# r3fang/alignTools.C

Measured on AMD Instinct MI355X. Metric: GCUPS (DP cell updates/s), SW affine-gap 150bp pairs, higher is better.
Workload: dtype int16; 1 GPU; C2: local affine-gap, 100000 x (150x150 bp) pairs per GPU, uniform ACGT, m=2 u=-2 o=-5 e=-2, scores+tracebacks+rendered strings; pairs_per_gpu=100000, l1=150, l2=150, bits_per_base=2, streams=3, parallelism=pairs sharded over 1 GPU(s), one process per GPU

## Files before the change

### aligntools/c_amd/csrc/at_hip.hip

```cpp
#include "at_launch.h"
#include "at_classes.h"
#include "at_ragplan.h"
#include "at_pack.hip.h"
#include "at_render.hip.h"
#include "at_myers.hip.h"
#include "at_search.hip.h"
#include "at_revcomp.hip.h"
#include "at_cigar.hip.h"
#include "at_edit_tb.hip.h"
#include "../../../include/aligntools_hip.h"

#include <algorithm>
#include <chrono>
#include <condition_variable>
#include <mutex>
#include <cstdarg>
#include <cstdio>
#include <cstdlib>
#include <cstring>
#include <functional>
#include <string>
#include <thread>
#include <vector>

// ... 475 lines not shown
		L.g = 16;
		L.k = at::class_rows(at::kClass16, l1);
	} else if ((force_g == 16 || (!force_g && g_forced != 64 && g_forced != 32)) && ts == 4 && l1 > 208 && l1 <= at::class_top(at::kClass16)) {
		L.g = 16;
		L.k = at::class_rows(at::kClass16, l1);
	} else if (g_forced != 64 && ts == 4 && l1 > 208 &&
	           l1 <= (force_g || g_forced == 32 ? at::kTopFit : kmode == at::K_LOCAL ? at::kTopLocal : kmode == at::K_GLOBAL ? at::kTopGlobal : at::kTopFit)) {
		L.g = 32;
		L.k = at::class_rows(at::kClass32, l1, 0, g_forced == 32 ? at::kClass32SkipUnderGroup32 : 0);
	}
	const int ng = 64 / L.g;
	const int blk = L.g <= 16 ? 4 : 8;
	const int tbk = (l2 + L.g - 1 + blk - 1) / blk;
	L.ptr_lanes = L.g == 64 ? std::max(1, std::min(64, (l1 + L.k - 1) / L.k)) : 64;
	L.ptr_lanes = (L.ptr_lanes + 3) & ~3;
	const long long nstrips = (l1 + L.g * L.k - 1) / (L.g * L.k);
	long long nref = (at::kPad + (long long)tbk * blk) / 4 + 4;
	nref = (nref + 1) & ~1LL;
	const long long walk_words = ((L.k + 3) / 4 + (hasj ? ((L.k + 3) / 4 + 3) / 4 : 0)) * (long long)at::ck_steps(L.g);
	const long long nbound = std::max<long long>(2LL * (l2 + 2), two_pass == 1 ? std::max<long long>(at::ck_stage_words(at::ck_steps(L.g)), 2 * ng * walk_words * (L.g == 64 ? 4 : 1)) : 0);
	const int spw = overlap ? 16 / AT_OVL_BITS : (hasj && !(ts == 4 && AT_JPLANE)) ? 2 : 4;
	const long long njpl = tb && hasj && ts == 4 && AT_JPLANE ? nstrips * tbk * (blk / 4) * ((L.k + 3) / 4) * L.ptr_lanes : 0;
	const long long nptr = tb ? nstrips * tbk * (blk / spw) * L.k * L.ptr_lanes + njpl + 64 : 0;
	const long long nsm = hasj ? (((long long)l2 + 64 + 64 + 128 + 31) / 32 + 2 + 1) & ~1LL : 0;
	L.off_refb = (int)nref;
	L.off_bound = (int)(2 * nref * ng);
	L.off_sm = (int)(2 * nref * ng + nbound);
	L.nsm = (int)nsm;
	L.off_ptr = (int)((2 * nref * ng + nbound + nsm + 3) & ~3LL);
	L.words = L.off_ptr + nptr;
	return L;
}

static bool packed_ok(const at_handle *h, int mode, int bits, int l1, int l2, int ts, int *thresh16)
{
	const long long scale = 1LL << ts;
	if (getenv("AT_NO_PACKED") && atoi(getenv("AT_NO_PACKED"))) return false;
	if ((bits != 2 && bits != 8) || l1 < 1 || l2 < 1) return false;
	if (mode == AT_MODE_OVERLAP) {
		if (ts != 2 || h->m < 0 || h->u > 0 || h->o > 0) return false;
		const long long lo = std::llabs((long long)h->o) * std::max(l1, l2) + std::llabs((long long)h->u) + 16;
		const long long hi = (long long)h->m * std::min(l1, l2), slack = std::llabs((long long)h->o) + std::llabs((long long)h->u) + 3;
		if (scale * (lo + hi + slack) >= 32768) return false;
		*thresh16 = (int)(-32768 + scale * (hi + slack));
		return true;
	}
	if (!(mode == AT_MODE_GLOBAL || mode == AT_MODE_LOCAL || mode == AT_MODE_FIT)) return false;
	if (h->m < 0 || h->u > 0 || h->o > 0 || h->e > 0) return false;
	const bool hasj = mode == AT_MODE_FIT && h->use_jump;
	if (hasj && (h->j > 0 || std::llabs((long long)h->j - h->o) * scale > 32000)) return false;
	const long long A = std::max<long long>(std::max(std::llabs((long long)h->e), std::llabs((long long)h->u)), h->m);
	(void)A;
	long long lo = 3 * std::llabs((long long)h->o) + (hasj ? std::llabs((long long)h->j) : 0) +
	               std::llabs((long long)h->u) * std::min(l1, l2) + std::llabs((long long)h->e) * std::max(l1, l2) + 16;
	if (mode == AT_MODE_LOCAL) lo = std::llabs((long long)h->o) + std::llabs((long long)h->u) + std::llabs((long long)h->e) + 16;
	const long long hi = (long long)h->m * std::min(l1, l2);
	const long long slack = std::llabs((long long)h->o) + std::llabs((long long)h->e) + 3;
	if (scale * (lo + hi + slack) >= 32768) return false;
	*thresh16 = (int)(-32768 + scale * (hi + slack));
	return true;
}

struct TpLayout {
	int off_brow, off_rck, off_cck, off_rptr, off_rjpl;
	long long words;
	long long brow_words;
};
static TpLayout tp_layout(const Layout16 &L, int kmode, int l2, bool split = false)
{
	const int blk = L.g <= 16 ? 4 : 8, cb = at::ck_steps(L.g);
	const long long T = (long long)((l2 + L.g - 1 + blk - 1) / blk) * blk;
	const int es = 2, nq = ((kmode == at::K_FITJ ? 3 : 2) * L.k + 3) / 4, kg = (L.k + 3) / 4;
	auto up4 = [](long long v) { return (v + 3) & ~3LL; };
	TpLayout t;
	long long w = 0;
	t.brow_words = (T + cb + 2) * es;
	t.off_brow = (int)w; if (!split) w = up4(w + (T + cb + 2) * es);
	t.off_rck = (int)w; w = up4(w + 64 * es + (T / cb + 3) * 64 * cb * es);
	t.off_cck = (int)w; w = up4(w + (T / cb + 3) * ((nq + AT_CK_COL_QUAD - 1) / AT_CK_COL_QUAD * AT_CK_COL_QUAD) * 256);
	t.off_rptr = (int)w; if (!split) w = up4(w + (cb / 4) * ((L.k + 3) / 4) * 256);
	t.off_rjpl = (int)w; if (!split) w = up4(w + (cb / 4) * ((kg + 3) / 4) * 256);
	t.words = split ? (w + 63) & ~63LL : w;
	return t;
}

static int choose_store(long long words_fixed, long long words_ptr, bool prefer_hbm_pointers);
static bool packed16_kernel_exists(int kmode, const Layout16 &P, bool tb, int ts, int bits, int rag, const Layout16 *PT = nullptr)
{
	const long long fixed = PT ? std::max(P.off_ptr, PT->off_ptr) : P.off_ptr;
	const long long ptrw = PT ? std::max(P.words - P.off_ptr, PT->words - PT->off_ptr) : P.words - P.off_ptr;
	const int st = choose_store(fixed, ptrw, P.g < 64 || rag);
// ... 298 lines not shown
	drop_stale_error();

	long long maxabs = 0;
	for (int v : {h->m, h->u, h->o, h->e, h->j}) maxabs = std::max<long long>(maxabs, std::llabs((long long)v));
	maxabs = std::max<long long>(maxabs, 1);
	if (maxabs * ((long long)max_len1 + max_len2 + 2) >= (1LL << 24))
		return fail(h, AT_ERR_RANGE, "scores may exceed the exact range: max|param|=%lld, l1+l2=%lld", maxabs,
		            (long long)max_len1 + max_len2);

	h->last_span = max_len1 + max_len2;
	const int kmode = mode == AT_MODE_GLOBAL ? at::K_GLOBAL : mode == AT_MODE_LOCAL ? at::K_LOCAL
	                : mode == AT_MODE_FIT ? (h->use_jump ? at::K_FITJ : at::K_FIT)
	                : mode == AT_MODE_OVERLAP ? at::K_OVERLAP : at::K_EDIT;

	int thresh16 = 0, ts = 0;
	if (!uniform_shape && !rag && !only_if && ap_n == 0 && npairs >= 4096 && !d_order && kmode <= at::K_FITJ &&
	    env_ll("AT_AUTO_UNIFORM", 1) && (bits == 8 || scores_fit_byte(h, mode)) &&
	    packed_ok(h, mode, bits, max_len1, max_len2, 4, &thresh16)) {
		int *flag = h->d_rflag + 8;
		HIP_TRY(h, hipMemsetAsync(flag, 0xff, 4, stream));
		const unsigned cg = (unsigned)std::min<int64_t>((npairs + 255) / 256, 4LL * h->ncu);
		hipLaunchKernelGGL(at::at_check_uniform, dim3(cg), dim3(256), 0, stream, d_len1, d_len2, (long long)npairs, max_len1, max_len2, flag);
		int rc = align_device(h, mode, npairs, d_seq, bits, d_woff1, d_len1, d_woff2, d_len2, max_len1, max_len2, 1, want_traceback,
		                      d_score, d_end_i, d_end_j, d_state, d_ops, d_ops_off, d_nops, stream_, 0, 0, nullptr, 0, flag, -1);
		if (rc) return rc;
		std::string packed_cfg = h->cfg;
		rc = align_device(h, mode, npairs, d_seq, bits, d_woff1, d_len1, d_woff2, d_len2, max_len1, max_len2, 0, want_traceback,
		                  d_score, d_end_i, d_end_j, d_state, d_ops, d_ops_off, d_nops, stream_, 0, 0, nullptr, 0, flag, 0);
		if (rc) return rc;
		snprintf(h->cfg, sizeof h->cfg, "auto: [%.140s] if every pair is %dx%d, else [%.120s]", packed_cfg.c_str(), max_len1, max_len2,
		         std::string(h->cfg).c_str());
		return AT_OK;
	}
	if ((uniform_shape || rag) && ap_n == 0) {
		if (packed_ok(h, mode, bits, max_len1, max_len2, 4, &thresh16)) ts = 4;
		else if ((!rag || kmode == at::K_OVERLAP) && packed_ok(h, mode, bits, max_len1, max_len2, 2, &thresh16)) ts = 2;
		if (kmode == at::K_OVERLAP && (!tb || getenv("AT_NO_PACKED_OVERLAP"))) ts = 0;
	}
	if (rag && (!ts || (kmode > at::K_FITJ && !(kmode == at::K_OVERLAP && rag == 64)) || max_len1 > at::rag_group_top(rag) || !d_order))
		return fail(h, AT_ERR_ARG, "ragged packed launch outside its domain");
	Layout16 P;
	if (ts) {
		P = layout16_for(tb, kmode == at::K_FITJ, max_len1, max_len2, ts, rag, kmode == at::K_OVERLAP, kmode,
		                 rag && kmode == at::K_OVERLAP ? at::class_rows(at::kClassOvl, max_len1) : 0);
		const double min_rounds = getenv("AT_PACKED_MIN_ROUNDS") ? atof(getenv("AT_PACKED_MIN_ROUNDS")) : 1.0;
		if (!rag && P.g == 64 && (double)((npairs + 1) / 2) < min_rounds * 12.0 * h->ncu) ts = 0;
		if (P.words >= (1LL << 24)) { if (rag) return fail(h, AT_ERR_ARG, "ragged packed launch outside its domain (slot too large)"); ts = 0; }
		Layout16 PTq = P;
		const bool tailq = !rag && !only_if && P.g <= 16 && kmode != at::K_OVERLAP && env_ll("AT_TAIL_SPLIT", 1);
		if (tailq) PTq = layout16_for(tb, kmode == at::K_FITJ, max_len1, max_len2, ts, at::AT_TAIL_G, false, kmode, at::at_tail_k(P.g, P.k));
		if (ts && !packed16_kernel_exists(kmode, P, tb, ts, bits, rag, tailq ? &PTq : nullptr)) {
			if (rag) return fail(h, AT_ERR_ARG, "ragged packed launch outside its domain (frame too long for LDS)");
			ts = 0;
		}
	}
	bool two_pass = false;
	int tp_split = 0;
	const char *ck_note = "";
	const long long tp_mode = env_ll("AT_TWO_PASS", 1);
	if (ts && tb && !rag && kmode <= at::K_FITJ && tp_mode) {
		Layout16 P2 = layout16_for(false, kmode == at::K_FITJ, max_len1, max_len2, ts, 0, false, kmode, 0, 1);
		const bool narrow_default = P2.g == 8 && tp_split_narrow_default(kmode, max_len1, max_len2);
		const bool split_default = P2.g == 64 || narrow_default;
		const bool split_want = env_ll("AT_TP_SPLIT", split_default ? 1 : 0) && at_pick_walk16(kmode, P2.g, P2.k, ts, bits);
		const int split_req = split_want && !h->ck_alloc_failed && !h->ck_skip ? 1 : 0;
		if (split_want && !split_req) ck_note = h->ck_skip ? " [one work item's checkpoints exceed AT_CK_CAP_MB: no separate pass 2]"
		                                                   : " [checkpoint buffer unavailable on this handle: no separate pass 2]";
		if ((P2.g == 64 || tp_mode >= 2 || (split_req && narrow_default)) && (long long)P2.g * P2.k >= max_len1 && at_pick16_tp(kmode, P2.g, P2.k, ts, bits) &&
		    choose_store(P2.off_ptr, 1, true) == 1) {
			two_pass = true;
			tp_split = split_req;
			if (tp_split) P2 = layout16_for(false, kmode == at::K_FITJ, max_len1, max_len2, ts, 0, false, kmode, 0, 2);
			P = P2;
		}
	}
	if (ts) {
		const int per_wave = 2 * (64 / P.g);
		const bool tail_ok = !rag && !only_if && P.g <= 16 && kmode != at::K_OVERLAP && env_ll("AT_TAIL_SPLIT", 1) &&
		                     (!tp_split || P.g == 8);
		Layout16 PT = P;
		if (tail_ok) PT = layout16_for(tb && !two_pass, kmode == at::K_FITJ, max_len1, max_len2, ts, at::AT_TAIL_G, false, kmode, at::at_tail_k(P.g, P.k), two_pass ? (tp_split ? 2 : 1) : 0);
		TpLayout tpm{}, tpt{};
		if (two_pass) { tpm = tp_layout(P, kmode, max_len2, tp_split != 0); tpt = tp_layout(PT, kmode, max_len2, tp_split != 0); }
		int64_t piece = npairs;
		int64_t brow_words = 0;
		if (tp_split) {
			const long long cap = env_ll("AT_CK_CAP_MB", 8192) << 20;
			brow_words = (tpm.brow_words + 63) & ~63LL;
			const long long tail_reserve = tail_ok ? 16LL * h->ncu * tpt.words * 4 : 0;
			const long long items = (cap - tail_reserve - brow_words * 4) / (tpm.words * 4 + 16LL * per_wave);
			if (items < 1) {
				struct SkipForThisCall {
					at_handle *h;
					explicit SkipForThisCall(at_handle *hh) : h(hh) { h->ck_skip = true; }
					~SkipForThisCall() { h->ck_skip = false; }
				} skip(h);
				return align_device(h, mode, npairs, d_seq, bits, d_woff1, d_len1, d_woff2, d_len2, max_len1, max_len2, uniform_shape, want_traceback,
				                    d_score, d_end_i, d_end_j, d_state, d_ops, d_ops_off, d_nops, stream_, ap_n, ap_first, d_order, rag, only_if, only_val);
			}
			piece = std::min<int64_t>(npairs, items * per_wave);
			const long long forced = env_ll("AT_CK_PIECE_PAIRS", 0);
			if (forced > 0) piece = std::min<int64_t>(piece, std::max<long long>(1, forced / per_wave) * per_wave);
		}
		auto walk_lane_words = [&](const Layout16 &L) -> long long {
			const int cb = at::ck_steps(L.g);
			return L.k * (cb / 4) + (kmode == at::K_FITJ ? (L.k + 3) / 4 * (cb / 4) : 0);
		};
// ... 485 lines not shown
		HIP_TRY(h, hipGetLastError());
		return AT_OK;
	};
	const size_t b_len1 = al((size_t)npairs * 4);
	const size_t b_ops = al((size_t)ops_total + 64), b_pfx = al((size_t)(npairs + 1) * 8);
	const size_t out_need = 5 * b_len1 + b_ops + (tb ? b_pfx : 0);
	rc = grow(h, &h->d_out, &h->out_bytes, out_need);
	if (rc) return rc;
	char *dout = (char *)h->d_out;
	int32_t *d_score = (int32_t *)dout, *d_ei = (int32_t *)(dout + b_len1), *d_ej = (int32_t *)(dout + 2 * b_len1);
	int32_t *d_st = (int32_t *)(dout + 3 * b_len1), *d_nops = (int32_t *)(dout + 4 * b_len1);
	uint8_t *d_ops = (uint8_t *)(dout + 5 * b_len1);
	int64_t *d_poff = (int64_t *)(dout + 5 * b_len1 + b_ops);

	int *d_order = nullptr;
	bool frames = false;
	const bool ragged = !uniform && npairs > 1 && npairs < (1LL << 31);
	if (!ragged) {
		rc = settle_alphabet();
		if (rc) return rc;
	}
	if (ragged) {
		int th = 0, min1 = INT32_MAX, min2 = INT32_MAX;
		for (int64_t k = 0; k < npairs; ++k) { min1 = std::min(min1, len1[k]); min2 = std::min(min2, len2[k]); }
		const bool affine = mode == AT_MODE_LOCAL || mode == AT_MODE_GLOBAL || mode == AT_MODE_FIT;
		const bool ovl = mode == AT_MODE_OVERLAP && tb;
		const int kmode_f = mode == AT_MODE_LOCAL ? at::K_LOCAL : mode == AT_MODE_GLOBAL ? at::K_GLOBAL : mode == AT_MODE_OVERLAP ? at::K_OVERLAP
		                  : h->use_jump ? at::K_FITJ : at::K_FIT;
		const int64_t min_bucket = env_ll("AT_RAGGED_MIN_BUCKET", 16384);
		at::RagPlan plan;
		for (int pass = 0; pass < 2; ++pass) {
			const int planned_bits = bits;
			frames = (affine || ovl) && max1 <= at::one_strip_top(mode) && min1 >= 1 && min2 >= 1 && npairs >= 64 && env_ll("AT_RAGGED_PACKED", 1) &&
			         packed_ok(h, mode, bits, max1, max2, ovl ? 2 : 4, &th);
			if (frames) {
				const bool hasj = kmode_f == at::K_FITJ;
				const int tsf = ovl ? 2 : 4;
				int prev = -1;
				for (int gq : at::kRagGroups) {
					const int l1q = std::min(max1, at::rag_group_top(gq));
					if (!frames || (ovl && gq != 64) || l1q < min1 || l1q == prev) continue;
					prev = l1q;
					const at::GroupRows c = at::rag_class(mode, ovl, l1q);
					frames = packed16_kernel_exists(kmode_f, layout16_for(tb, hasj, l1q, max2, tsf, c.g, ovl, kmode_f, ovl ? c.k : 0), tb, tsf, bits, c.g);
				}
			}
			plan = at::rag_plan(mode, ovl, len1, len2, npairs, max1, max2, min_bucket, frames);
			if (pass == 0) {
				rc = settle_alphabet();
				if (rc) return rc;
			}
			if (bits == planned_bits) break;
		}
		htrace("chunk: planned, pair", pair_base);
		const std::vector<int> &order = plan.order;
		rc = grow(h, &h->d_order, &h->order_bytes, order.size() * 4);
		if (rc) return rc;
		rc = grow_pinned(h, &h->hp_order, &h->hp_order_bytes, order.size() * 4);
		if (rc) return rc;
		memcpy(h->hp_order, order.data(), order.size() * 4);
		d_order = (int *)h->d_order;
		HIP_TRY(h, hipMemcpyAsync(d_order, h->hp_order, order.size() * 4, hipMemcpyHostToDevice, s));
		for (const at::RagLaunch &L : plan.launches) {
			rc = align_device(h, mode, L.b1 - L.b0, d_words, bits, d_woff1, d_len1, d_woff2, d_len2, L.f1, L.f2, 0, tb ? 1 : 0,
			                  d_score, d_ei, d_ej, d_st, tb ? d_ops : nullptr, tb ? d_opsoff : nullptr, tb ? d_nops : nullptr, s,
			                  0, 0, d_order + L.b0, L.g);
			if (rc) return rc;
// ... 743 lines not shown
```

### aligntools/c_amd/csrc/at_sweep16.hip.h

```cpp
#pragma once
#include "at_sweep.hip.h"
#include <utility>

#ifndef AT_WALK_AHEAD
#define AT_WALK_AHEAD 4
#endif
#ifndef AT_DIAG_NO_WALK
#define AT_DIAG_NO_WALK 0
#endif
#ifndef AT_GLOBAL_WALK_AHEAD
#define AT_GLOBAL_WALK_AHEAD 1
#endif
#ifndef AT_LOCAL_WALK_AHEAD
#define AT_LOCAL_WALK_AHEAD 1
#endif
#ifndef AT_WALK_PRIO
#define AT_WALK_PRIO 2
#endif
#ifndef AT_JPLANE
#define AT_JPLANE 1
#endif
#ifndef AT_OVL_BITS
#define AT_OVL_BITS 2
#endif
// ... 17 lines not shown
	const long long *ops_off;
	int *nops;
	uint32_t *ws;
	long long ws_slot_words;
	int off_refb, off_bound, off_ptr, off_sm, nsm;
	int ptr_lanes;
	unsigned long long *queue;
	const int *order;
	const int *only_if;
	int only_val;
	int off_brow, off_rck, off_cck, off_rptr, off_rjpl;
	uint32_t *ck;
	long long ck_item_words;
	uint32_t *ck_brow;
	int4 *tp_end;
};

AT_DEV uint32_t pk2(int v) { return ((uint32_t)v & 0xffffu) | ((uint32_t)v << 16); }
AT_DEV uint32_t pminu(uint32_t a, uint32_t b)
{
	uint32_t d;
	asm("v_pk_min_u16 %0, %1, %2" : "=v"(d) : "v"(a), "v"(b));
	return d;
}
AT_DEV uint32_t pmad(uint32_t a, uint32_t b, uint32_t c)
{
	uint32_t d;
	asm("v_pk_mad_i16 %0, %1, %2, %3" : "=v"(d) : "v"(a), "v"(b), "v"(c));
	return d;
}
AT_DEV uint32_t padd(uint32_t a, uint32_t b)
{
	return __builtin_bit_cast(uint32_t, __builtin_elementwise_add_sat(__builtin_bit_cast(s16x2, a), __builtin_bit_cast(s16x2, b)));
}
AT_DEV uint32_t psub(uint32_t a, uint32_t b)
{
	return __builtin_bit_cast(uint32_t, __builtin_elementwise_sub_sat(__builtin_bit_cast(s16x2, a), __builtin_bit_cast(s16x2, b)));
}
AT_DEV uint32_t pmax(uint32_t a, uint32_t b)
{
	return __builtin_bit_cast(uint32_t, __builtin_elementwise_max(__builtin_bit_cast(s16x2, a), __builtin_bit_cast(s16x2, b)));
}
AT_DEV uint32_t pshl4(uint32_t a)
{
	return __builtin_bit_cast(uint32_t, __builtin_bit_cast(s16x2, a) << (s16x2)(4));
}
template <int N>
AT_DEV uint32_t pshln(uint32_t a)
{
	return __builtin_bit_cast(uint32_t, __builtin_bit_cast(s16x2, a) << (s16x2)(N));
}
AT_DEV uint32_t pshl8(uint32_t a)
{
	return __builtin_bit_cast(uint32_t, __builtin_bit_cast(s16x2, a) << (s16x2)(8));
}
AT_DEV uint32_t pneg(uint32_t a)
{
	return __builtin_bit_cast(uint32_t, __builtin_bit_cast(s16x2, a) >> (s16x2)(15));
}
AT_DEV int half(uint32_t v, int h) { return (int)(short)(h ? (v >> 16) : (v & 0xffffu)); }

constexpr uint32_t kClean2 = 0xfff0fff0u, kTagL2 = 0x000f000fu, kTagM2 = 0x000a000au, kTagU2 = 0x00010001u;
constexpr int kNeg16 = -32768;

template <int MODE>
AT_DEV void border16(int i, int j, int o16, int e16, int &L, int &M, int &U)
// ... 401 lines not shown
	static_assert(!TP || (!TB && !RAG && MODE != K_OVERLAP && !PTRLDS), "two-pass tracebacks: uniform batches of the affine modes, checkpoints in the global slot");
	static_assert(BITS == 2 || BITS == 8, "sequence words: 16 two-bit codes or 4 bytes");
	static_assert(!RAG || G <= 32 || MODE == K_OVERLAP, "ragged frames: one strip (the host sizes the frame for it)");
	static_assert(MODE == K_GLOBAL || MODE == K_LOCAL || MODE == K_FIT || MODE == K_FITJ || MODE == K_OVERLAP, "packed path: the affine modes, overlap");
	constexpr bool OVL = MODE == K_OVERLAP;
	static_assert(!OVL || (TB && TS == 2), "packed overlap: scores x4 with 2-bit tags, tracebacks");
	constexpr bool HASJ = MODE == K_FITJ;
	constexpr bool ISFIT = MODE == K_FIT || MODE == K_FITJ;
	static_assert(TS == 4 || TS == 2, "scores x16 or x4");
	constexpr int TMASK = (1 << TS) - 1;
	constexpr int CS = TMASK + 1, NCH = (K + CS - 1) / CS;
	constexpr int OTGL = TS == 4 ? 15 : 3, OTGM = TS == 4 ? 10 : 2, OTGU = 1;
	constexpr int TGL = TB ? OTGL : 0, TGM = TB ? OTGM : 0, TGU = TB ? OTGU : 0;
	constexpr bool JPL = HASJ && TB && TS == 4 && AT_JPLANE;
	constexpr int KG = (K + 3) / 4;
	constexpr int PB = OVL ? AT_OVL_BITS : (HASJ && !JPL) ? 8 : 4;
	static_assert(!OVL || G == 64, "packed overlap: one 64-lane group");
	constexpr int SPW = 16 / PB;
	static_assert(G == 64 || G == 32 || G == 16 || G == 8 || G == 4, "group width");
	constexpr int NG = 64 / G;
	constexpr int BLK = G <= 16 ? 4 : 8;
	constexpr bool ONEBODY = G <= 16 || (CK > 0 && AT_TP_ONEBODY);
	constexpr int RPB = BLK / SPW;
	constexpr int RS = G * K;
	constexpr int PADW = kPad / 4;
	const int lane = threadIdx.x;
	const int grp = lane / G, lg = lane % G;
	Slot<SMALL> mem;
	mem.g = SMALL ? nullptr : a.ws + (long long)blockIdx.x * a.ws_slot_words;
	PtrStore<PTRLDS> pm;
	pm.g = PTRLDS ? nullptr : a.ws + (long long)blockIdx.x * a.ws_slot_words;
	const int l1 = a.l1, l2 = a.l2, NL = a.ptr_lanes;
	const int o16 = a.o16, e16 = a.e16;
	uint32_t o2 = pk2(a.o16), e2 = pk2(a.e16);
	const int mS = OVL ? a.m16 | 2 : a.m16, uS = OVL ? a.u16 | 2 : a.u16;
	uint32_t lut_lo = ((uint32_t)mS & 0xffu) | (((uint32_t)uS & 0xffu) * 0x01010100u);
	uint32_t lut_hi = (((uint32_t)mS >> 8) & 0xffu) | ((((uint32_t)uS >> 8) & 0xffu) * 0x01010100u);
	uint32_t oL2 = pk2(a.o16 | 3), oR2 = pk2(a.o16 | 1);
	asm volatile("" : "+v"(oL2), "+v"(oR2));
	uint32_t cClean = (uint32_t)(0xffff & ~TMASK) * 0x00010001u, cTagM = (uint32_t)TGM * 0x00010001u;
	uint32_t cTagL = (uint32_t)TGL * 0x00010001u, cTagU = (uint32_t)TGU * 0x00010001u;
	uint32_t cM3 = 0x00030003u, cM7 = 0x00070007u, cNib = 0x000f000fu, cF0 = 0x00f000f0u, cF000 = 0xf000f000u;
	uint32_t c8888 = 0x88888888u, c3333 = 0x33333333u;
	asm volatile("" : "+v"(c8888), "+v"(c3333));
	uint32_t cRTagL = (uint32_t)OTGL * 0x00010001u, cRTagM = (uint32_t)OTGM * 0x00010001u, cRTagU = (uint32_t)OTGU * 0x00010001u;
	(void)cRTagL; (void)cRTagM; (void)cRTagU;
	if constexpr (CK > 0) asm volatile("" : "+v"(cRTagL), "+v"(cRTagM), "+v"(cRTagU));
	uint32_t gmo2 = pk2(a.g16 - a.o16), neg2 = 0x80008000u;
	asm volatile("" : "+v"(gmo2), "+v"(neg2));
	uint32_t c1 = 0x00010001u, umm2 = pk2(a.u16 - a.m16), m2 = pk2(mS);
	asm volatile("" : "+v"(c1), "+v"(umm2), "+v"(m2));
	asm volatile("" : "+v"(o2), "+v"(e2), "+v"(lut_lo), "+v"(lut_hi));
	asm volatile("" : "+v"(cClean), "+v"(cTagM), "+v"(cTagL), "+v"(cTagU), "+v"(cM3), "+v"(cM7), "+v"(cNib), "+v"(cF0), "+v"(cF000));
	const int nstrips = (l1 + RS - 1) / RS;
	const int tbk_frame = (l2 + G - 1 + BLK - 1) / BLK;
	const int wps = tbk_frame * RPB * K;
	const int wpj = tbk_frame * (BLK / 4) * KG;
	const int jpl_base0 = a.off_ptr + __mul24(nstrips * wps, NL);
	const long long nwork = (a.npairs + 2 * NG - 1) / (2 * NG);
	const int refoff = grp * 2 * a.off_refb;
	uint32_t *gs = TP ? a.ws + (long long)blockIdx.x * a.ws_slot_words : nullptr;
	constexpr int ES = ck_es<MODE>();
	const int ck_T = tbk_frame * BLK;
	(void)gs; (void)ck_T;
	if constexpr (TP) {
		uint32_t *const brow = SPLIT ? a.ck_brow : gs + a.off_brow;
		for (int j = lane; j <= l2; j += 64) {
			int L, M, U;
// ... 54 lines not shown
			}
		}
		const int tbk = RAG ? (il2 + G - 1 + BLK - 1) / BLK : tbk_frame;
		const int lastlane = il1 > 0 ? ((il1 - 1) % RS) / K : 0;
		const int rl = il1 > 0 ? ((il1 - 1) % RS) % K : 0;
		const uint32_t *qA = a.seq + a.woff1[pA], *qB = a.seq + a.woff1[pB];
		const uint32_t *rA = a.seq + a.woff2[pA], *rB = a.seq + a.woff2[pB];

		{
			constexpr int BPW = 32 / BITS;
			const int nw2 = (il2 + BPW - 1) / BPW;
			const int nwA = (l2A + BPW - 1) / BPW, nwB = (l2B + BPW - 1) / BPW;
			for (int w = lg; w < nw2; w += G) {
				const uint32_t va = rA[RAG ? imin(w, nwA - 1) : w], vb = rB[RAG ? imin(w, nwB - 1) : w];
				if constexpr (BITS == 8) {
					mem.st(refoff + PADW + w, va);
					mem.st(refoff + a.off_refb + PADW + w, vb);
				} else {
#pragma unroll
					for (int q = 0; q < 4; ++q) {
						const uint32_t ba = (va >> (8 * q)) & 0xffu, bb = (vb >> (8 * q)) & 0xffu;
						mem.st(refoff + PADW + 4 * w + q, (ba & 3u) | ((ba & 0xcu) << 6) | ((ba & 0x30u) << 12) | ((ba & 0xc0u) << 18));
						mem.st(refoff + a.off_refb + PADW + 4 * w + q, (bb & 3u) | ((bb & 0xcu) << 6) | ((bb & 0x30u) << 12) | ((bb & 0xc0u) << 18));
					}
				}
			}
		}
		if constexpr (HASJ) {
			for (int w = lane; w < a.nsm; w += 64) mem.st(a.off_sm + w, a.sitemask[w]);
		}
		for (int j = lane; j <= l2; j += 64) {
			int L, M, U;
			border16<MODE>(0, j, o16, e16, L, M, U);
			int x = imax3(L | TGL, M | TGM, U | TGU);
			const int ld = imax(sat16((L | TGL) + e16), sat16((M | TGM) + o16));
			if constexpr (OVL) x = j == 0 ? 0 : kNeg16;
			mem.st2(a.off_bound + 2 * j, pk2(x), pk2(ld));
		}
		mem.sync();

		int gbi[2] = {INT32_MAX, INT32_MAX}, gbj[2] = {INT32_MAX, INT32_MAX}, gbs[2] = {INT32_MIN, INT32_MIN};
		uint32_t bestM = pk2(a.thresh16), bestMj = 0, bestL = pk2(a.thresh16), bestLj = 0;
		uint32_t capL = 0, capM = 0, capU = 0;
		uint32_t Mo_l[K], U_l[K], Xl[2][K], L_l[K], J_l[K];
		uint32_t Lrow = 0;

		for (int s = 0; s < nstrips; ++s) {
			const int base = s * RS;
			const int i0 = base + lg * K;
			const int nl = imin(G, (il1 - base + K - 1) / K);
			const bool laststrip = s == nstrips - 1;
			const bool wb = G == 64 && !laststrip;
			uint32_t qsel[K], acc[K], keymask[K];
			uint32_t accH[OVL && PB == 2 ? K : 1];
			uint32_t jA[JPL ? KG : 1], jB[JPL ? KG : 1];
			(void)accH; (void)jA; (void)jB;
			if constexpr (JPL) {
#pragma unroll
				for (int g = 0; g < KG; ++g) { jA[g] = 0; jB[g] = 0; }
			}
			const int jpl_base = jpl_base0 + __mul24(s * wpj, NL);
#pragma unroll
			for (int r = 0; r < K; ++r) {
				const int qi = imin(i0 + r, l1A - 1), qj = imin(i0 + r, l1B - 1);
				uint32_t ca, cb;
				if constexpr (BITS == 2) { ca = (qA[qi >> 4] >> ((qi & 15) * 2)) & 3u; cb = (qB[qj >> 4] >> ((qj & 15) * 2)) & 3u; }
				else { ca = (qA[qi >> 2] >> ((qi & 3) * 8)) & 0xffu; cb = (qB[qj >> 2] >> ((qj & 3) * 8)) & 0xffu; }
				qsel[r] = (ca * 0x00000101u + cb * 0x01010000u) | (BITS == 2 ? 0x04000400u : 0u);
				acc[r] = 0;
				keymask[r] = (i0 + r < l1A ? (uint32_t)(0xffff & ~TMASK) : 0u) | (i0 + r < l1B ? (uint32_t)(0xffff & ~TMASK) << 16 : 0u);
				int L, M, U;
				border16<MODE>(i0 + r + 1, 0, o16, e16, L, M, U);
				L = sat16(L);
				Mo_l[r] = pk2(sat16((M | TGM) + o16));
				U_l[r] = pk2(U | TGU);
				L_l[r] = pk2(L | TGL);
				if constexpr (ISFIT) Lrow = L_l[r];
				J_l[r] = neg2;
				Xl[0][r] = pk2(imax3(L | TGL, M | TGM, U | TGU));
				if constexpr (OVL) Xl[0][r] = 0;
				Xl[1][r] = Xl[0][r];
			}
			uint32_t ckL = 0, ckM = 0, ckU = 0, ckJ = neg2;
			int ck_p = 0;
			(void)ckL; (void)ckM; (void)ckU; (void)ckJ; (void)ck_p;
			if constexpr (TP) {
				int L, M, U;
				border16<MODE>(i0 + K, 0, o16, e16, L, M, U);
				ckL = pk2(sat16(L)); ckM = pk2(M); ckU = pk2(U);
				const int p0 = a.off_rck + ck_rck_word<ES>(0, lane);
				const uint2 en = ck_entry<HASJ>(ckL, ckM, ckU, ckJ, e2, o2, cRTagL, cRTagM, cRTagU);
				gs[p0] = en.x; gs[p0 + 1] = en.y;
			}
			uint32_t A_prev = Xl[0][K - 1], B_prev = 0, Ad;
			{
				int L, M, U;
				border16<MODE>(base, 0, o16, e16, L, M, U);
				L = sat16(L);
				Ad = pk2(imax3(L | TGL, M | TGM, U | TGU));
				if constexpr (OVL) Ad = 0;
			}
			uint32_t best[NCH], bt[NCH];
#pragma unroll
			for (int c = 0; c < NCH; ++c) { best[c] = 0x80008000u; bt[c] = 0; }
			auto load_bound = [&](int t0, uint32_t &bx, uint32_t &bl) {
				const int jn = imin(t0 + 1 + (lane & (BLK - 1)), l2);
				const uint2 v = mem.ld2(a.off_bound + 2 * jn);
				bx = v.x; bl = v.y;
			};
			uint32_t bx, bl, bxn, bln;
			load_bound(0, bx, bl);
			const int ptr_base = a.off_ptr + s * wps * NL;

			for (int blk = 0; blk < tbk; ++blk) {
				const int t0 = blk * BLK;
				if constexpr (TP) ck_p = a.off_rck + ck_rck_word<ES>(t0 + 1, lane);
				load_bound(t0 + BLK, bxn, bln);
				uint32_t wA[2], wB[2];
				{
					const int e0 = t0 - lg + kPad;
					const int w = refoff + (e0 >> 2);
					const int sh = (e0 & 3) * 8;
					const uint32_t a0 = mem.ld(w), a1 = mem.ld(w + 1);
					const uint32_t b0 = mem.ld(a.off_refb + w), b1 = mem.ld(a.off_refb + w + 1);
					wA[0] = __builtin_amdgcn_alignbit(a1, a0, sh);
					wB[0] = __builtin_amdgcn_alignbit(b1, b0, sh);
					wA[1] = 0; wB[1] = 0;
					if constexpr (BLK == 8) {
						const uint32_t a2 = mem.ld(w + 2), b2 = mem.ld(a.off_refb + w + 2);
						wA[1] = __builtin_amdgcn_alignbit(a2, a1, sh);
						wB[1] = __builtin_amdgcn_alignbit(b2, b1, sh);
					}
				}
				uint32_t sm = 0;
				if constexpr (HASJ) {
					const int e0 = t0 - lg + 1 + 64;
					const uint32_t w0 = mem.ld(a.off_sm + (e0 >> 5)), w1 = mem.ld(a.off_sm + (e0 >> 5) + 1);
// ... 5 lines not shown
					constexpr int k = decltype(KC)::value;
					constexpr bool masked = decltype(MASKED)::value;
					constexpr int kk = k & 3, hw = k >> 2;
					constexpr uint32_t SELK = (uint32_t)kk * 0x00000101u + (uint32_t)(4 + kk) * 0x01010000u;
					const int t = t0 + k;
					uint32_t tpk = pk2(t);
					asm("" : "+v"(tpk));
					const uint32_t Aup = grp_up1<G>((uint32_t)row_shl<k>((int)bx), A_prev);
					const uint32_t Bup = grp_up1<G>((uint32_t)row_shl<k>((int)bl), B_prev);
					const int jm1 = jm1_0 + k;
					bool active = true;
					if constexpr (masked) active = lg < nl && (unsigned)jm1 < (unsigned)il2;
					if (active) {
						uint32_t gopen = neg2;
						if constexpr (HASJ) gopen = ((sm >> k) & 1u) ? gmo2 : neg2;
						if constexpr (OVL) {
							if (laststrip) {
								const uint32_t jpk = pk2(jm1);
								uint32_t vM = pick<K>(Xl[k & 1], rl);
								if constexpr (RAG) {
									const uint32_t cm = (((uint32_t)((jm1 - l2A) >> 31)) & 0xffffu) | (((uint32_t)((jm1 - l2B) >> 31)) << 16);
									vM = vbfi(cm, vM, neg2);
								}
								uint32_t dM = psub(bestM, vM);
								asm("" : "+v"(dM));
								bestMj = vbfi(pneg(dM), jpk, bestMj); bestM = pmax(bestM, vM);
							}
						}
						if constexpr (ISFIT) {
							if (laststrip) {
								const uint32_t jpk = pk2(jm1);
								uint32_t vM = psub(pick<K>(Mo_l, rl), o2);
								uint32_t vL = Lrow;
								if constexpr (RAG) {
									const uint32_t cm = (((uint32_t)((jm1 - l2A) >> 31)) & 0xffffu) | (((uint32_t)((jm1 - l2B) >> 31)) << 16);
									vM = vbfi(cm, vM, neg2); vL = vbfi(cm, vL, neg2);
								}
								uint32_t dM = psub(bestM, vM);
								asm("" : "+v"(dM));
								bestMj = vbfi(pneg(dM), jpk, bestMj); bestM = pmax(bestM, vM);
								uint32_t dL = psub(bestL, vL);
								asm("" : "+v"(dL));
								bestLj = vbfi(pneg(dL), jpk, bestLj); bestL = pmax(bestL, vL);
							}
						}
						const uint32_t selw = __builtin_amdgcn_perm(wB[hw], wA[hw], SELK);
						uint32_t diag = Ad, lraw = Bup, up = 0, cmax[NCH];
						uint32_t capmask = 0;
						if constexpr (RAG && MODE == K_GLOBAL) {
							if (lg == lastlane) capmask = (jm1 + 1 == l2A ? 0xffffu : 0u) | (jm1 + 1 == l2B ? 0xffff0000u : 0u);
						}
						uint32_t upv = Aup;
						uint32_t jn = 0;
						(void)jn;
#pragma unroll
						for (int r = 0; r < K; ++r) {
							uint32_t S;
							if constexpr (BITS == 2) {
								S = __builtin_amdgcn_perm(lut_hi, lut_lo, selw ^ qsel[r]);
							} else {
								const uint32_t z = pminu(selw ^ qsel[r], c1);
								S = pmad(z, umm2, m2);
							}
							if constexpr (OVL) {
								const uint32_t left = Xl[k & 1][r];
								const uint32_t x = pmax(pmax(padd(left, oL2), padd(diag, S)), padd(upv, oR2));
								const uint32_t Mcl = x & cClean;
								constexpr int sw = k % SPW;
								if constexpr (PB == 4) {
									if constexpr (sw == 0) acc[r] = x;
									else if constexpr (sw == 1) acc[r] = __builtin_amdgcn_perm(x, acc[r], 0x06020400u);
									else if constexpr (sw == 2) acc[r] = vbfi(cF0, pshln<4>(x), acc[r]);
									else acc[r] = vbfi(cF000, pshln<12>(x), acc[r]);
								} else {
									if constexpr (sw == 0) acc[r] = x;
									else if constexpr (sw == 1) acc[r] = __builtin_amdgcn_perm(x, acc[r], 0x06020400u);
									else if constexpr (sw == 2) acc[r] = vbfi(cF0, pshln<4>(x), acc[r]);
									else if constexpr (sw == 3) acc[r] = vbfi(cF000, pshln<12>(x), acc[r]);
									else if constexpr (sw == 4) accH[r] = x;
									else if constexpr (sw == 5) accH[r] = __builtin_amdgcn_perm(x, accH[r], 0x06020400u);
									else if constexpr (sw == 6) accH[r] = vbfi(cF0, pshln<4>(x), accH[r]);
									else accH[r] = vbfi(cF000, pshln<12>(x), accH[r]);
								}
								diag = left;
								upv = Mcl;
								up = Mcl;
								Xl[(k & 1) ^ 1][r] = Mcl;
								continue;
							}
							uint32_t Mraw = padd(diag, S);
							if constexpr (MODE == K_LOCAL) Mraw = pmax(Mraw, 0u);
							const uint32_t Mc = TB ? vandor(Mraw, cClean, cTagM) : Mraw;
							const uint32_t Lc = TB ? (lraw | cTagL) : lraw;
							const uint32_t Uraw = pmax(Mo_l[r], padd(U_l[r], e2));
							const uint32_t Uc = TB ? vandor(Uraw, cClean, cTagU) : Uraw;
							const uint32_t Mo = padd(Mc, o2);
							uint32_t Xo = pmax(pmax(Lc, Mc), Uc);
							uint32_t Jraw = 0;
							if constexpr (HASJ) {
								Jraw = pmax(padd(Mo_l[r], gopen), J_l[r]);
								const uint32_t Jc = TB ? (Jraw & cClean) : Jraw;
								Xo = pmax(Xo, Jc);
								J_l[r] = Jc;
							}
							const uint32_t Ld = pmax(padd(Lc, e2), Mo);
							if (TP && r == K - 1) {
								ckL = Lc; ckM = Mc; ckU = Uc;
								if constexpr (HASJ) ckJ = J_l[r];
							}
							if constexpr (RAG && MODE == K_GLOBAL) {
								if (r == rl) { capL = vbfi(capmask, Lc, capL); capM = vbfi(capmask, Mc, capM); capU = vbfi(capmask, Uc, capU); }
							}
							if constexpr (TB) {
								uint32_t c;
								if constexpr (TS == 4) {
									c = vbfi(cM7, vbfi(cM3, Mraw, lraw), Uraw);
								} else {
									c = vbfi(cM7, vbfi(cM3, Mraw, pshln<2>(lraw)), pshln<3>(Uraw));
								}
								if constexpr (HASJ && !JPL) c = vbfi(cNib, c, pshln<TS == 4 ? 1 : 3>(Jraw));
								if constexpr (JPL) {
									const int q = r & 3, gq = r >> 2;
									if (q == 0) jn = Jraw;
									else if (q == 1) jn = __builtin_amdgcn_perm(Jraw, jn, 0x06020400u);
									else if (q == 2) jn = vbfi(cF0, pshln<4>(Jraw), jn);
									else jn = vbfi(cF000, pshln<12>(Jraw), jn);
									if (q == 3 || r == K - 1) {
										if (q == 0) jn &= 0x000f000fu; else if (q == 1) jn &= 0x0f0f0f0fu; else if (q == 2) jn &= 0x0fff0fffu;
										constexpr int sj = k & 3;
										if constexpr (sj == 0) jA[gq] = jn;
										else if constexpr (sj == 1) jA[gq] = vbfi(c8888, jn, jA[gq]);
										else if constexpr (sj == 2) jB[gq] = jn;
										else jB[gq] = vbfi(c8888, jn, jB[gq]);
									}
								}
								constexpr int sw = k % SPW;
								if constexpr (sw == 0) acc[r] = c;
								else if constexpr (sw == 1) acc[r] = __builtin_amdgcn_perm(c, acc[r], 0x06020400u);
								else if constexpr (sw == 2) acc[r] = vbfi(cF0, pshln<4>(c), acc[r]);
								else acc[r] = vbfi(cF000, pshln<12>(c), acc[r]);
							}
							if constexpr (MODE == K_LOCAL) {
								uint32_t rt = (uint32_t)(TMASK - r % CS) * 0x00010001u;
								const uint32_t key = (Mraw & keymask[r]) | rt;
								cmax[r / CS] = r % CS == 0 ? key : pmax(cmax[r / CS], key);
							}
							diag = Xl[k & 1][r];
							Xl[(k & 1) ^ 1][r] = Xo;
							lraw = Ld;
							up = Xo;
							Mo_l[r] = Mo; U_l[r] = Uc;
							if constexpr (MODE == K_GLOBAL) L_l[r] = Lc;
							if constexpr (ISFIT) Lrow = r == rl ? Lc : Lrow;
						}
						if constexpr (MODE == K_LOCAL) {
							if constexpr (RAG) {
								const uint32_t cm = (((uint32_t)((jm1 - l2A) >> 31)) & 0xffffu) | (((uint32_t)((jm1 - l2B) >> 31)) << 16);
#pragma unroll
								for (int c = 0; c < NCH; ++c) cmax[c] = vbfi(cm, cmax[c], neg2);
							}
#pragma unroll
							for (int c = 0; c < NCH; ++c) {
								uint32_t dlt = psub(best[c], cmax[c]);
								asm("" : "+v"(dlt));
								const uint32_t g = pneg(dlt);
								bt[c] = vbfi(g, tpk, bt[c]);
								best[c] = pmax(best[c], cmax[c]);
							}
						}
						A_prev = up; B_prev = lraw;
						if (wb && lane == 63) mem.st2(a.off_bound + 2 * (jm1 + 1), up, lraw);
					}
					Ad = Aup;
					if constexpr (TP) {
						static_assert(!TP || AT_CK_ROW_TILE <= 1 || BLK % AT_CK_ROW_TILE == 0 || AT_CK_ROW_TILE % BLK == 0, "a tile of row checkpoints and a block of steps: one holds the other");
						constexpr int RT = AT_CK_ROW_TILE > 1 ? AT_CK_ROW_TILE : 1;
						constexpr int so = RT >= BLK ? k * ES : (k / RT) * 64 * RT * ES + (k % RT) * ck_rck_step<ES>();
						*(uint2 *)(gs + ck_p + so) = ck_entry<HASJ>(ckL, ckM, ckU, ckJ, e2, o2, cRTagL, cRTagM, cRTagU);
					}
					if constexpr (TB) {
						if constexpr (OVL && PB == 2) {
							if constexpr ((k + 1) % SPW == 0) {
#pragma unroll
								for (int r = 0; r < K; ++r) acc[r] = vbfi(c3333, acc[r], accH[r] << 2);
							}
						}
						if ((k + 1) % SPW == 0 && lane < NL) {
							if constexpr (PTRLDS) {
#pragma unroll
								for (int r = 0; r < K; ++r) pm.st(ptr_base + pidx<true, K>(blk * RPB + k / SPW, r, lane, NL), acc[r]);
							} else {
								const int wr = blk * RPB + k / SPW;
#pragma unroll
								for (int r = 0; r + 3 < K; r += 4)
									pm.st4(ptr_base + pidx<false, K>(wr, r, lane, NL), acc[r], acc[r + 1], acc[r + 2], acc[r + 3]);
								constexpr int R4 = K / 4 * 4;
								if constexpr (K - R4 == 3) {
									pm.st(ptr_base + pidx<false, K>(wr, R4, lane, NL), acc[R4]);
									pm.st(ptr_base + pidx<false, K>(wr, R4 + 1, lane, NL), acc[R4 + 1]);
									pm.st(ptr_base + pidx<false, K>(wr, R4 + 2, lane, NL), acc[R4 + 2]);
								} else if constexpr (K - R4 == 2) {
									pm.st2(ptr_base + pidx<false, K>(wr, R4, lane, NL), acc[R4], acc[R4 + 1]);
								} else if constexpr (K - R4 == 1) {
									pm.st(ptr_base + pidx<false, K>(wr, R4, lane, NL), acc[R4]);
								}
							}
// ... 87 lines not shown
			for (int h = 0; h < 2; ++h) {
				int bs = gbs[h], bi = gbi[h], bj = gbj[h];
				for (int d = G / 2; d >= 1; d >>= 1) {
					const int ob = __shfl_xor(bs, d), oi = __shfl_xor(bi, d), oj = __shfl_xor(bj, d);
					const bool take = ob > bs || (ob == bs && (oi < bi || (oi == bi && oj < bj)));
					if (take) { bs = ob; bi = oi; bj = oj; }
				}
				gbs[h] = bs; gbi[h] = bi; gbj[h] = bj;
			}
		}
		{
			const int h = lane & 1;
			const int glane = (lane >> 1) * G;
			const int own = (glane + lastlane) & 63;
			int sc16 = 0, ci = 0, cj = 0, st = 2;
			bool ok = true;
			auto from = [&](uint32_t v, int src) { return (uint32_t)__shfl((int)v, src & 63); };
			if constexpr (MODE == K_LOCAL) {
				const int s0 = (int)from((uint32_t)gbs[0], glane), s1 = (int)from((uint32_t)gbs[1], glane);
				const int i0 = (int)from((uint32_t)gbi[0], glane), i1 = (int)from((uint32_t)gbi[1], glane);
				const int j0 = (int)from((uint32_t)gbj[0], glane), j1 = (int)from((uint32_t)gbj[1], glane);
				sc16 = h ? s1 : s0; ci = h ? i1 : i0; cj = h ? j1 : j0;
				st = 2;
			} else if constexpr (MODE == K_GLOBAL) {
				int eL, eM, eU;
				if constexpr (RAG) {
					eL = half(from(capL, own), h);
					eM = half(from(capM, own), h);
					eU = half(from(capU, own), h);
					const int ca = (int)from((uint32_t)l2A, glane), cb = (int)from((uint32_t)l2B, glane);
					cj = h ? cb : ca;
				} else {
					eL = half(from(pick<K>(L_l, rl), own), h);
					eM = half(psub(from(pick<K>(Mo_l, rl), own), pk2(o16)), h);
					eU = half(from(pick<K>(U_l, rl), own), h);
					cj = l2;
				}
				const int x = TB ? imax3(eL, eM, eU) : imax3(eL | OTGL, eM | OTGM, eU | OTGU);
				sc16 = x; st = x & 3; ci = il1;
			} else if constexpr (OVL) {
				sc16 = half(from(bestM, own), h);
				cj = half(from(bestMj, own), h);
				ci = il1; st = 2;
				ok = sc16 > a.thresh16;
			} else {
				const int bM = half(from(bestM, own), h);
				const int jM = half(from(bestMj, own), h);
				const int bL = half(from(bestL, own), h);
				const int jL = half(from(bestLj, own), h);
				ci = il1;
				if ((bL >> TS) > (bM >> TS) && bL > a.thresh16) { sc16 = bL; st = 3; cj = jL; }
				else { sc16 = bM; st = 2; cj = jM; }
				ok = sc16 > a.thresh16;
			}
			my_sc = sc16; my_ci = ci; my_cj = cj; my_st = st; my_ok = ok;
		}
		if constexpr (TP && SPLIT) {
			const long long pin = wk * 2 * NG + lane;
			if (lane < 2 * NG && pin < a.npairs) {
				a.score[pin] = my_ok ? (my_sc >> TS) : INT32_MIN;
				if (a.end_i) a.end_i[pin] = my_ci;
				if (a.end_j) a.end_j[pin] = my_cj;
				if (a.state) a.state[pin] = my_st == 3 ? 1 : my_st == 2 ? 2 : 3;
				a.tp_end[pin] = make_int4(my_ci, my_cj, my_st, my_ok ? 1 : 0);
			}
		} else if constexpr (TP) {
			constexpr int LCB = ck_log2(CK);
			constexpr int KG2 = (K + 3) / 4;
			const int g2 = lane >> 1, h = lane & 1;
			const long long pin = wk * 2 * NG + lane;
			const bool mine = lane < 2 * NG && pin < a.npairs;
			int ci = my_ci, cj = my_cj, st = my_st, cnt = 0;
// ... 373 lines not shown
```

Before: 3193 GCUPS.

## Use column-drifted score representation to drop gap-extend add from inner recurrence

Rewrites the packed int16 affine-gap sweep for local, global and fit modes so that scores are stored offset by -e times the column index. In this representation the vertical gap extension becomes a plain max, and the horizontal one is a single add applied after the max. The offset is folded into the match/mismatch LUT, the gap-open constant, the borders and the local-mode zero floor through a per-column drift term, and it is removed again when the final score is reported. The host now checks that the drifted values still fit in int16, retrying the layout selection with a stricter bound when needed. This trims packed ALU ops per cell, but adds a per-column dcol update and extra subtractions in the local max-tracking, and it can force fallback to wider paths for long sequences.

```diff
diff --git a/aligntools/c_amd/csrc/at_hip.hip b/aligntools/c_amd/csrc/at_hip.hip
--- a/aligntools/c_amd/csrc/at_hip.hip
+++ b/aligntools/c_amd/csrc/at_hip.hip
@@ -531,7 +531,7 @@
 	return L;
 }
 
-static bool packed_ok(const at_handle *h, int mode, int bits, int l1, int l2, int ts, int *thresh16)
+static bool packed_ok(const at_handle *h, int mode, int bits, int l1, int l2, int ts, int *thresh16, bool drifted = false)
 {
 	const long long scale = 1LL << ts;
 	if (getenv("AT_NO_PACKED") && atoi(getenv("AT_NO_PACKED"))) return false;
@@ -556,6 +556,7 @@
 	const long long hi = (long long)h->m * std::min(l1, l2);
 	const long long slack = std::llabs((long long)h->o) + std::llabs((long long)h->e) + 3;
 	if (scale * (lo + hi + slack) >= 32768) return false;
+	if (drifted && !hasj && scale * (hi + std::llabs((long long)h->e) * l2 + slack) >= 32768) return false;
 	*thresh16 = (int)(-32768 + scale * (hi + slack));
 	return true;
 }
@@ -920,47 +921,55 @@
 		         std::string(h->cfg).c_str());
 		return AT_OK;
 	}
-	if ((uniform_shape || rag) && ap_n == 0) {
-		if (packed_ok(h, mode, bits, max_len1, max_len2, 4, &thresh16)) ts = 4;
-		else if ((!rag || kmode == at::K_OVERLAP) && packed_ok(h, mode, bits, max_len1, max_len2, 2, &thresh16)) ts = 2;
-		if (kmode == at::K_OVERLAP && (!tb || getenv("AT_NO_PACKED_OVERLAP"))) ts = 0;
-	}
-	if (rag && (!ts || (kmode > at::K_FITJ && !(kmode == at::K_OVERLAP && rag == 64)) || max_len1 > at::rag_group_top(rag) || !d_order))
-		return fail(h, AT_ERR_ARG, "ragged packed launch outside its domain");
+	const bool drift_mode = kmode == at::K_LOCAL || kmode == at::K_GLOBAL || kmode == at::K_FIT;
 	Layout16 P;
-	if (ts) {
-		P = layout16_for(tb, kmode == at::K_FITJ, max_len1, max_len2, ts, rag, kmode == at::K_OVERLAP, kmode,
-		                 rag && kmode == at::K_OVERLAP ? at::class_rows(at::kClassOvl, max_len1) : 0);
-		const double min_rounds = getenv("AT_PACKED_MIN_ROUNDS") ? atof(getenv("AT_PACKED_MIN_ROUNDS")) : 1.0;
-		if (!rag && P.g == 64 && (double)((npairs + 1) / 2) < min_rounds * 12.0 * h->ncu) ts = 0;
-		if (P.words >= (1LL << 24)) { if (rag) return fail(h, AT_ERR_ARG, "ragged packed launch outside its domain (slot too large)"); ts = 0; }
-		Layout16 PTq = P;
-		const bool tailq = !rag && !only_if && P.g <= 16 && kmode != at::K_OVERLAP && env_ll("AT_TAIL_SPLIT", 1);
-		if (tailq) PTq = layout16_for(tb, kmode == at::K_FITJ, max_len1, max_len2, ts, at::AT_TAIL_G, false, kmode, at::at_tail_k(P.g, P.k));
-		if (ts && !packed16_kernel_exists(kmode, P, tb, ts, bits, rag, tailq ? &PTq : nullptr)) {
-			if (rag) return fail(h, AT_ERR_ARG, "ragged packed launch outside its domain (frame too long for LDS)");
-			ts = 0;
-		}
-	}
 	bool two_pass = false;
 	int tp_split = 0;
 	const char *ck_note = "";
-	const long long tp_mode = env_ll("AT_TWO_PASS", 1);
-	if (ts && tb && !rag && kmode <= at::K_FITJ && tp_mode) {
-		Layout16 P2 = layout16_for(false, kmode == at::K_FITJ, max_len1, max_len2, ts, 0, false, kmode, 0, 1);
-		const bool narrow_default = P2.g == 8 && tp_split_narrow_default(kmode, max_len1, max_len2);
-		const bool split_default = P2.g == 64 || narrow_default;
-		const bool split_want = env_ll("AT_TP_SPLIT", split_default ? 1 : 0) && at_pick_walk16(kmode, P2.g, P2.k, ts, bits);
-		const int split_req = split_want && !h->ck_alloc_failed && !h->ck_skip ? 1 : 0;
-		if (split_want && !split_req) ck_note = h->ck_skip ? " [one work item's checkpoints exceed AT_CK_CAP_MB: no separate pass 2]"
-		                                                   : " [checkpoint buffer unavailable on this handle: no separate pass 2]";
-		if ((P2.g == 64 || tp_mode >= 2 || (split_req && narrow_default)) && (long long)P2.g * P2.k >= max_len1 && at_pick16_tp(kmode, P2.g, P2.k, ts, bits) &&
-		    choose_store(P2.off_ptr, 1, true) == 1) {
-			two_pass = true;
-			tp_split = split_req;
-			if (tp_split) P2 = layout16_for(false, kmode == at::K_FITJ, max_len1, max_len2, ts, 0, false, kmode, 0, 2);
-			P = P2;
-		}
+	for (int bound_pass = 0; bound_pass < 2; ++bound_pass) {
+		const bool drifted = drift_mode && (rag || bound_pass == 1);
+		ts = 0; two_pass = false; tp_split = 0; ck_note = "";
+		if ((uniform_shape || rag) && ap_n == 0) {
+			if (packed_ok(h, mode, bits, max_len1, max_len2, 4, &thresh16, drifted)) ts = 4;
+			else if ((!rag || kmode == at::K_OVERLAP) && packed_ok(h, mode, bits, max_len1, max_len2, 2, &thresh16, drifted)) ts = 2;
+			if (kmode == at::K_OVERLAP && (!tb || getenv("AT_NO_PACKED_OVERLAP"))) ts = 0;
+		}
+		if (rag && (!ts || (kmode > at::K_FITJ && !(kmode == at::K_OVERLAP && rag == 64)) || max_len1 > at::rag_group_top(rag) || !d_order))
+			return fail(h, AT_ERR_ARG, "ragged packed launch outside its domain");
+		if (ts) {
+			P = layout16_for(tb, kmode == at::K_FITJ, max_len1, max_len2, ts, rag, kmode == at::K_OVERLAP, kmode,
+			                 rag && kmode == at::K_OVERLAP ? at::class_rows(at::kClassOvl, max_len1) : 0);
+			const double min_rounds = getenv("AT_PACKED_MIN_ROUNDS") ? atof(getenv("AT_PACKED_MIN_ROUNDS")) : 1.0;
+			if (!rag && P.g == 64 && (double)((npairs + 1) / 2) < min_rounds * 12.0 * h->ncu) ts = 0;
+			if (P.words >= (1LL << 24)) { if (rag) return fail(h, AT_ERR_ARG, "ragged packed launch outside its domain (slot too large)"); ts = 0; }
+			Layout16 PTq = P;
+			const bool tailq = !rag && !only_if && P.g <= 16 && kmode != at::K_OVERLAP && env_ll("AT_TAIL_SPLIT", 1);
+			if (tailq) PTq = layout16_for(tb, kmode == at::K_FITJ, max_len1, max_len2, ts, at::AT_TAIL_G, false, kmode, at::at_tail_k(P.g, P.k));
+			if (ts && !packed16_kernel_exists(kmode, P, tb, ts, bits, rag, tailq ? &PTq : nullptr)) {
+				if (rag) return fail(h, AT_ERR_ARG, "ragged packed launch outside its domain (frame too long for LDS)");
+				ts = 0;
+			}
+		}
+		const long long tp_mode = env_ll("AT_TWO_PASS", 1);
+		if (ts && tb && !rag && kmode <= at::K_FITJ && tp_mode) {
+			Layout16 P2 = layout16_for(false, kmode == at::K_FITJ, max_len1, max_len2, ts, 0, false, kmode, 0, 1);
+			const bool narrow_default = P2.g == 8 && tp_split_narrow_default(kmode, max_len1, max_len2);
+			const bool split_default = P2.g == 64 || narrow_default;
+			const bool split_want = env_ll("AT_TP_SPLIT", split_default ? 1 : 0) && at_pick_walk16(kmode, P2.g, P2.k, ts, bits);
+			const int split_req = split_want && !h->ck_alloc_failed && !h->ck_skip ? 1 : 0;
+			if (split_want && !split_req) ck_note = h->ck_skip ? " [one work item's checkpoints exceed AT_CK_CAP_MB: no separate pass 2]"
+			                                                   : " [checkpoint buffer unavailable on this handle: no separate pass 2]";
+			if ((P2.g == 64 || tp_mode >= 2 || (split_req && narrow_default)) && (long long)P2.g * P2.k >= max_len1 && at_pick16_tp(kmode, P2.g, P2.k, ts, bits) &&
+			    choose_store(P2.off_ptr, 1, true) == 1) {
+				two_pass = true;
+				tp_split = split_req;
+				if (tp_split) P2 = layout16_for(false, kmode == at::K_FITJ, max_len1, max_len2, ts, 0, false, kmode, 0, 2);
+				P = P2;
+			}
+		}
+		const bool one_pass_drifted = ts && !two_pass && drift_mode;
+		int th = 0;
+		if (drifted || !one_pass_drifted || packed_ok(h, mode, bits, max_len1, max_len2, ts, &th, true)) break;
 	}
 	if (ts) {
 		const int per_wave = 2 * (64 / P.g);
@@ -1512,7 +1521,7 @@
 		for (int pass = 0; pass < 2; ++pass) {
 			const int planned_bits = bits;
 			frames = (affine || ovl) && max1 <= at::one_strip_top(mode) && min1 >= 1 && min2 >= 1 && npairs >= 64 && env_ll("AT_RAGGED_PACKED", 1) &&
-			         packed_ok(h, mode, bits, max1, max2, ovl ? 2 : 4, &th);
+			         packed_ok(h, mode, bits, max1, max2, ovl ? 2 : 4, &th,  true);
 			if (frames) {
 				const bool hasj = kmode_f == at::K_FITJ;
 				const int tsf = ovl ? 2 : 4;
diff --git a/aligntools/c_amd/csrc/at_sweep16.hip.h b/aligntools/c_amd/csrc/at_sweep16.hip.h
--- a/aligntools/c_amd/csrc/at_sweep16.hip.h
+++ b/aligntools/c_amd/csrc/at_sweep16.hip.h
@@ -73,6 +73,11 @@
 AT_DEV uint32_t padd(uint32_t a, uint32_t b)
 {
 	return __builtin_bit_cast(uint32_t, __builtin_elementwise_add_sat(__builtin_bit_cast(s16x2, a), __builtin_bit_cast(s16x2, b)));
+}
+AT_DEV uint32_t paddw(uint32_t a, uint32_t b)
+{
+	typedef unsigned short u16x2 __attribute__((ext_vector_type(2)));
+	return __builtin_bit_cast(uint32_t, (u16x2)(__builtin_bit_cast(u16x2, a) + __builtin_bit_cast(u16x2, b)));
 }
 AT_DEV uint32_t psub(uint32_t a, uint32_t b)
 {
@@ -540,8 +545,11 @@
 	pm.g = PTRLDS ? nullptr : a.ws + (long long)blockIdx.x * a.ws_slot_words;
 	const int l1 = a.l1, l2 = a.l2, NL = a.ptr_lanes;
 	const int o16 = a.o16, e16 = a.e16;
-	uint32_t o2 = pk2(a.o16), e2 = pk2(a.e16);
-	const int mS = OVL ? a.m16 | 2 : a.m16, uS = OVL ? a.u16 | 2 : a.u16;
+	constexpr bool DRIFT = CK == 0 && (MODE == K_LOCAL || MODE == K_GLOBAL || MODE == K_FIT);
+	const int oe16 = DRIFT ? o16 - e16 : o16;
+	uint32_t o2 = pk2(oe16), e2 = pk2(a.e16);
+	const uint32_t ne2 = pk2(-a.e16);
+	const int mS = OVL ? a.m16 | 2 : a.m16 - (DRIFT ? e16 : 0), uS = OVL ? a.u16 | 2 : a.u16 - (DRIFT ? e16 : 0);
 	uint32_t lut_lo = ((uint32_t)mS & 0xffu) | (((uint32_t)uS & 0xffu) * 0x01010100u);
 	uint32_t lut_hi = (((uint32_t)mS >> 8) & 0xffu) | ((((uint32_t)uS >> 8) & 0xffu) * 0x01010100u);
 	uint32_t oL2 = pk2(a.o16 | 3), oR2 = pk2(a.o16 | 1);
@@ -662,6 +670,10 @@
 		for (int j = lane; j <= l2; j += 64) {
 			int L, M, U;
 			border16<MODE>(0, j, o16, e16, L, M, U);
+			if constexpr (DRIFT) {
+				const int dj = -e16 * j;
+				L = L == kNeg16 ? L : L + dj; M = M == kNeg16 ? M : M + dj; U = U == kNeg16 ? U : U + dj;
+			}
 			int x = imax3(L | TGL, M | TGM, U | TGU);
 			const int ld = imax(sat16((L | TGL) + e16), sat16((M | TGM) + o16));
 			if constexpr (OVL) x = j == 0 ? 0 : kNeg16;
@@ -702,7 +714,7 @@
 				int L, M, U;
 				border16<MODE>(i0 + r + 1, 0, o16, e16, L, M, U);
 				L = sat16(L);
-				Mo_l[r] = pk2(sat16((M | TGM) + o16));
+				Mo_l[r] = pk2(sat16((M | TGM) + oe16));
 				U_l[r] = pk2(U | TGU);
 				L_l[r] = pk2(L | TGL);
 				if constexpr (ISFIT) Lrow = L_l[r];
@@ -733,6 +745,8 @@
 			uint32_t best[NCH], bt[NCH];
 #pragma unroll
 			for (int c = 0; c < NCH; ++c) { best[c] = 0x80008000u; bt[c] = 0; }
+			uint32_t dcol = pk2(-e16 * ((MODE == K_LOCAL ? 1 : 0) - lg));
+			(void)dcol;
 			auto load_bound = [&](int t0, uint32_t &bx, uint32_t &bl) {
 				const int jn = imin(t0 + 1 + (lane & (BLK - 1)), l2);
 				const uint2 v = mem.ld2(a.off_bound + 2 * jn);
@@ -804,6 +818,7 @@
 								const uint32_t jpk = pk2(jm1);
 								uint32_t vM = psub(pick<K>(Mo_l, rl), o2);
 								uint32_t vL = Lrow;
+								if constexpr (DRIFT) { vM = psub(vM, dcol); vL = psub(vL, dcol); }
 								if constexpr (RAG) {
 									const uint32_t cm = (((uint32_t)((jm1 - l2A) >> 31)) & 0xffffu) | (((uint32_t)((jm1 - l2B) >> 31)) << 16);
 									vM = vbfi(cm, vM, neg2); vL = vbfi(cm, vL, neg2);
@@ -861,10 +876,10 @@
 								continue;
 							}
 							uint32_t Mraw = padd(diag, S);
-							if constexpr (MODE == K_LOCAL) Mraw = pmax(Mraw, 0u);
+							if constexpr (MODE == K_LOCAL) Mraw = pmax(Mraw, DRIFT ? dcol : 0u);
 							const uint32_t Mc = TB ? vandor(Mraw, cClean, cTagM) : Mraw;
 							const uint32_t Lc = TB ? (lraw | cTagL) : lraw;
-							const uint32_t Uraw = pmax(Mo_l[r], padd(U_l[r], e2));
+							const uint32_t Uraw = DRIFT ? pmax(Mo_l[r], U_l[r]) : pmax(Mo_l[r], padd(U_l[r], e2));
 							const uint32_t Uc = TB ? vandor(Uraw, cClean, cTagU) : Uraw;
 							const uint32_t Mo = padd(Mc, o2);
 							uint32_t Xo = pmax(pmax(Lc, Mc), Uc);
@@ -875,7 +890,7 @@
 								Xo = pmax(Xo, Jc);
 								J_l[r] = Jc;
 							}
-							const uint32_t Ld = pmax(padd(Lc, e2), Mo);
+							const uint32_t Ld = DRIFT ? padd(pmax(Lc, Mo), e2) : pmax(padd(Lc, e2), Mo);
 							if (TP && r == K - 1) {
 								ckL = Lc; ckM = Mc; ckU = Uc;
 								if constexpr (HASJ) ckJ = J_l[r];
@@ -933,6 +948,7 @@
 							}
 #pragma unroll
 							for (int c = 0; c < NCH; ++c) {
+								if constexpr (DRIFT) cmax[c] = psub(cmax[c], dcol);
 								uint32_t dlt = psub(best[c], cmax[c]);
 								asm("" : "+v"(dlt));
 								const uint32_t g = pneg(dlt);
@@ -944,6 +960,7 @@
 						if (wb && lane == 63) mem.st2(a.off_bound + 2 * (jm1 + 1), up, lraw);
 					}
 					Ad = Aup;
+					if constexpr (DRIFT && (MODE == K_LOCAL || MODE == K_FIT)) dcol = paddw(dcol, ne2);
 					if constexpr (TP) {
 						static_assert(!TP || AT_CK_ROW_TILE <= 1 || BLK % AT_CK_ROW_TILE == 0 || AT_CK_ROW_TILE % BLK == 0, "a tile of row checkpoints and a block of steps: one holds the other");
 						constexpr int RT = AT_CK_ROW_TILE > 1 ? AT_CK_ROW_TILE : 1;
@@ -1097,12 +1114,13 @@
 					cj = h ? cb : ca;
 				} else {
 					eL = half(from(pick<K>(L_l, rl), own), h);
-					eM = half(psub(from(pick<K>(Mo_l, rl), own), pk2(o16)), h);
+					eM = half(psub(from(pick<K>(Mo_l, rl), own), pk2(oe16)), h);
 					eU = half(from(pick<K>(U_l, rl), own), h);
 					cj = l2;
 				}
 				const int x = TB ? imax3(eL, eM, eU) : imax3(eL | OTGL, eM | OTGM, eU | OTGU);
-				sc16 = x; st = x & 3; ci = il1;
+				sc16 = DRIFT ? x + e16 * cj : x;
+				st = x & 3; ci = il1;
 			} else if constexpr (OVL) {
 				sc16 = half(from(bestM, own), h);
 				cj = half(from(bestMj, own), h);
```

Result: faster. 3264 GCUPS, median of 6 (+2.2%).
